# Bebra777228/PolGen-RVC

Hardware: AMD Instinct MI355X
Metric: real-time-factor (audio-sec/wall-sec) per GPU, 30s@16kHz RMVPE->48kHz (higher is better)
Workload: dtype f32 (conv products as 3 fp16 MFMAs of a hi/lo split, fp32 accumulate; fp32 elsewhere)

## Files before the change

### include/rvcx.h

```cpp
#ifndef RVCX_H
#define RVCX_H
#include <stdint.h>

#ifdef __cplusplus
extern "C" {
#endif

typedef struct rvcx_ctx rvcx_ctx;

typedef struct {
  const char* name;
  const void* data;
  int32_t dtype;
  int32_t ndim;
  int64_t shape[4];
} rvcx_tensor;

typedef struct {
  int32_t inter_channels, hidden_channels, filter_channels, n_heads, n_layers, kernel_size;
  int32_t n_resblocks;
  int32_t res_kernels[4];
  int32_t res_dilations[4][3];
  int32_t n_ups;
  int32_t up_rates[6], up_kernels[6];
// ... 242 lines not shown
int rvcx_index_features(rvcx_ctx*, int B, const float* wav_hd, int64_t n, int out_dim, float* feats_hd);
int64_t rvcx_kmeans_exhaustive(rvcx_ctx*);

int rvcx_debug_inject(rvcx_ctx*, int what);
double rvcx_flop_counter(rvcx_ctx*, int reset);
void* rvcx_stream(rvcx_ctx*);

int rvcx_op_fcpe_post(rvcx_ctx*, const float* raw_hd, int F_in, int p_len, double pitch, double f0_min, double f0_max,
                      int32_t* coarse, float* f0);
int rvcx_op_conv1d(rvcx_ctx*, const float* x, const float* w, const float* bias, const float* res,
                   float* y, int B, int Cin, int Tin, int Cout, int K, int stride, int dil,
                   int pad_left, int Tout, int groups, int pre_lrelu, float pre_slope, int act,
                   float act_slope, const int32_t* lens_in, const int32_t* lens_out);
int rvcx_op_resblock_pair(rvcx_ctx*, const float* x, const float* w1, const float* b1, const float* w2,
                          const float* b2, float* y, int B, int C, int T, int K, int dil, float slope, int fused,
                          const int32_t* lens);
int rvcx_op_resblock3(rvcx_ctx*, const float* x, const float* w1, const float* b1, const float* w2, const float* b2,
                      float* y, int B, int C, int T, const int32_t* dils, float slope, const int32_t* lens);
int rvcx_bench_resblock_pair(rvcx_ctx*, int B, int C, int T, int K, int dil, int fused, int iters,
                             float* ms_per_launch);
int rvcx_bench_conv1d(rvcx_ctx*, int B, int Cin, int Tin, int Cout, int K, int stride, int dil, int groups,
                      int iters, float* ms_per_launch);
int rvcx_conv_override(int tile, int variant, int splitk);
int rvcx_op_convtranspose1d(rvcx_ctx*, const float* x, const float* w, const float* bias, float* y,
                            int B, int Cin, int Tin, int Cout, int K, int stride, int pad,
                            int pre_lrelu, float pre_slope);
int rvcx_op_conv2d3x3(rvcx_ctx*, const float* x, const float* w, const float* bias, const float* res,
                      float* y, int B, int Cin, int H, int W, int Cout, int act);
int rvcx_op_convblock2d(rvcx_ctx*, const float* x, const float* w1, const float* b1, const float* w2, const float* b2,
                        const float* wsc, const float* bsc, float* y, int B, int Cin, int Cout, int H, int W,
                        const int32_t* rows);
int rvcx_op_convtranspose2d(rvcx_ctx*, const float* x, const float* w, const float* bias, float* y,
                            int B, int Cin, int H, int W, int Cout, int act);
int rvcx_op_attention(rvcx_ctx*, const float* q, const float* k, const float* v, float* out, int B,
                      int H, int D, int T, float scale, const float* emb_rel_k,
                      const float* emb_rel_v, int window, const int32_t* lens);
int rvcx_op_gemm_tm(rvcx_ctx*, const float* x_cf, const float* w, const float* bias, const float* res_tm, int B, int T,
                    int Cin, int Cout, int act, int exact_fp32, float* y_tm, float* y_cf, float* y_split);
int rvcx_bench_gemm(rvcx_ctx*, int64_t rows, int Cin, int Cout, int iters, float* ms_per_launch);
int rvcx_op_layernorm_tm(rvcx_ctx*, const float* x, const float* gamma, const float* beta, float* y, float* y_split,
                         int64_t rows, int C, float eps);
int rvcx_op_layernorm_c(rvcx_ctx*, const float* x, const float* gamma, const float* beta, float* y,
                        int B, int C, int T, float eps);
int rvcx_op_groupnorm_gelu(rvcx_ctx*, const float* x, const float* gamma, const float* beta, int B, int C, int T, float eps,
                           const int32_t* lens, float* y, float* stats, float* y_split);
int rvcx_op_hubert_conv0(rvcx_ctx*, const float* wav, const float* w, const float* gamma, const float* beta, int B, int C,
// ... 30 lines not shown
```

### polgen-rvc_amd/_lib.py

```python
from __future__ import annotations

import ctypes as C
import os
import threading
import types
from typing import Optional, Sequence

import numpy as np

_HERE = os.path.dirname(os.path.abspath(__file__))
LIB_PATH = os.environ.get("RVCX_LIBRARY") or os.path.join(_HERE, "librvcx.so")


class RvcxError(RuntimeError):
    pass


class Tensor(C.Structure):
    _fields_ = [("name", C.c_char_p), ("data", C.c_void_p), ("dtype", C.c_int32),
                ("ndim", C.c_int32), ("shape", C.c_int64 * 4)]


class SynthCfg(C.Structure):
    _fields_ = [("inter_channels", C.c_int32), ("hidden_channels", C.c_int32),
# ... 90 lines not shown
    Lb, Lx, Ls = int(Lb), int(Lx), int(Ls)
    assert y.shape == (Lb + Lx + Ls,) and b.shape == (Lx,)
    win = np.lib.stride_tricks.sliding_window_view(y[:Ls + Lx], Lx)
    den = np.sqrt((win * win).sum(1) + 1e-8)
    scores = (win @ b) / den
    mags = (np.abs(win) @ np.abs(b)) / den
    d = int(np.argmax(scores)) if offset is None else int(offset)
    out = y[d:d + Lb].copy()
    k = min(Lx, Lb)
    fin = np.sin(0.5 * np.pi * np.arange(Lx) / max(Lx - 1, 1)) ** 2
    out[:k] = y[d:d + k] * fin[:k] + b[:k] * (1.0 - fin[:k])
    return out, y[d + Lb:d + Lb + Lx].copy(), d, scores, mags


_lib = None

SYMBOLS = [
    "rvcx_create", "rvcx_destroy", "rvcx_last_error", "rvcx_version", "rvcx_load_hubert",
    "rvcx_load_rmvpe", "rvcx_index_exhaustive", "rvcx_load_crepe", "rvcx_crepe_frames", "rvcx_crepe_predict", "rvcx_op_crepe_decode", "rvcx_get_f0_crepe_x", "rvcx_load_fcpe", "rvcx_fcpe_f0", "rvcx_fcpe_frames", "rvcx_get_f0_fcpe_x", "rvcx_op_fcpe_post", "rvcx_load_synth", "rvcx_unload_synth", "rvcx_load_index", "rvcx_load_index_ivf",
    "rvcx_weights_regions", "rvcx_weights_adopt", "rvcx_weights_clone", "rvcx_rmvpe_f0", "rvcx_rmvpe_frames", "rvcx_rmvpe_mel", "rvcx_synth_infer_taps", "rvcx_hubert_features",
    "rvcx_hubert_frames", "rvcx_synth_infer", "rvcx_synth_infer_window", "rvcx_synth_dec_rf", "rvcx_synth_upp", "rvcx_index_blend",
    "rvcx_out_len", "rvcx_convert_batch", "rvcx_convert_batch_f64", "rvcx_micro_batch", "rvcx_bucket_length", "rvcx_last_micro_batches", "rvcx_last_cuts", "rvcx_noise_len",
    "rvcx_get_f0", "rvcx_get_f0_x", "rvcx_vc", "rvcx_vc_frames", "rvcx_last_timing",
    "rvcx_flop_counter", "rvcx_fp32_reruns", "rvcx_mem_info", "rvcx_conv_profile", "rvcx_conv_profile_csv", "rvcx_stream", "rvcx_op_conv1d", "rvcx_op_resblock_pair", "rvcx_bench_resblock_pair", "rvcx_bench_conv1d", "rvcx_conv_override", "rvcx_op_convtranspose1d",
    "rvcx_op_conv2d3x3", "rvcx_op_convblock2d", "rvcx_op_convtranspose2d", "rvcx_op_attention", "rvcx_op_layernorm_c",
    "rvcx_op_bigru", "rvcx_op_highpass", "rvcx_highpass_exact", "rvcx_convert_batch_ex", "rvcx_get_f0_x_ex", "rvcx_fp32_layers", "rvcx_fp32_pinned",
    "rvcx_gru_fallbacks", "rvcx_gru_publish_probe", "rvcx_debug_inject", "rvcx_f0_file_track", "rvcx_op_gemm_tm", "rvcx_op_layernorm_tm",
    "rvcx_resample_len", "rvcx_resample_f64", "rvcx_resample_f64_kind", "rvcx_bench_gemm", "rvcx_device_info",
    "rvcx_convert_submit", "rvcx_convert_wait", "rvcx_convert_poll", "rvcx_convert_inflight", "rvcx_ticket_lead_ms",
    "rvcx_synth_infer_head", "rvcx_op_sola", "rvcx_stream_open", "rvcx_stream_step", "rvcx_stream_reset", "rvcx_stream_close",
    "rvcx_stream_out_len", "rvcx_stream_noise_len", "rvcx_stream_frames",
    "rvcx_stream_open_io", "rvcx_stream_in_len", "rvcx_stream_delays", "rvcx_stream_resample_delay", "rvcx_stream_last_taps",
    "rvcx_stream_set", "rvcx_op_stream_resample",
    "rvcx_stream_open_fx", "rvcx_stream_out_channels", "rvcx_stream_set_fx", "rvcx_stream_last_fx_ms", "rvcx_op_stream_fx",
    "rvcx_fx_reverb_host",
    "rvcx_fx_chain", "rvcx_op_fx_highpass", "rvcx_op_fx_compressor", "rvcx_op_fx_gate", "rvcx_op_fx_reverb", "rvcx_op_fx_shelf",
    "rvcx_op_fx_chorus", "rvcx_op_fx_mix", "rvcx_fx_chunk", "rvcx_fx_last_passes", "rvcx_fx_cte", "rvcx_fx_delay",
    "rvcx_fx_coeffs", "rvcx_fx_highpass_host", "rvcx_fx_biquad_host", "rvcx_fx_follower_host", "rvcx_fx_compressor_host",
    "rvcx_fx_gate_host", "rvcx_fx_comb_host", "rvcx_fx_allpass_host", "rvcx_fx_chorus_host", "rvcx_fx_mix_host",
    "rvcx_op_groupnorm_gelu", "rvcx_op_hubert_conv0", "rvcx_op_sine_source", "rvcx_op_randn", "rvcx_op_reflect_pad",
    "rvcx_op_mel_post", "rvcx_op_decode_f0", "rvcx_op_avgpool2", "rvcx_op_gru_input", "rvcx_op_upsample_protect",
    "rvcx_kmeans", "rvcx_ivf_assign", "rvcx_kmeans_exhaustive", "rvcx_index_features",
    "rvcx_op_resblock3", "rvcx_flac_encode_bound", "rvcx_flac_encode_s16", "rvcx_flac_info", "rvcx_flac_decode_s32", "rvcx_flac_last_error",
]


def lib() -> C.CDLL:
# ... 530 lines not shown
    def resblock3(self, x, w1, b1, w2, b2, dils=(1, 3, 5), slope=0.1, lens=None):
        x, w1, w2 = f32(x), f32(w1), f32(w2)
        B, Cc, T = x.shape
        y = np.empty_like(x)
        b1 = None if b1 is None else f32(b1)
        b2 = None if b2 is None else f32(b2)
        d = i32(list(dils))
        li = i32(lens)
        self._ck(lib().rvcx_op_resblock3(self._h, _p(x), _p(w1), _p(b1), _p(w2), _p(b2), _p(y), B, Cc, T, _p(d, C.c_int32),
                                         C.c_float(slope), _p(li, C.c_int32)), "op_resblock3")
        return y

    def bench_resblock_pair(self, B, Cc, T, K, dil=1, fused=True, iters=10):
        ms = C.c_float(0)
        self._ck(lib().rvcx_bench_resblock_pair(self._h, B, Cc, T, K, dil, 1 if fused else 0, iters, C.byref(ms)),
                 "bench_resblock_pair")
        return ms.value, 4.0 * B * Cc * Cc * K * T / (ms.value * 1e-3) / 1e12

    @staticmethod
    def conv_override(tile=-1, variant=-1, splitk=-1):
        if lib().rvcx_conv_override(tile, variant, splitk) != 0:
            raise RvcxError("conv_override: " + (lib().rvcx_last_error(None) or b"").decode())

    def bench_conv1d(self, B, Cin, Tin, Cout, K, stride=1, dil=1, groups=1, iters=10):
        ms = C.c_float(0)
        self._ck(lib().rvcx_bench_conv1d(self._h, B, Cin, Tin, Cout, K, stride, dil, groups, iters, C.byref(ms)),
                 "bench_conv1d")
        pad = (K * dil - dil) // 2
        Tout = (Tin + 2 * pad - dil * (K - 1) - 1) // stride + 1
        flops = 2.0 * B * Cout * Tout * K * (Cin // groups)
        return ms.value, flops / (ms.value * 1e-3) / 1e12

    def convtranspose1d(self, x, w, bias=None, stride=1, pad=0, pre_lrelu=None):
        x, w = f32(x), f32(w)
        B, Cin, Tin = x.shape
        _, Cout, K = w.shape
        Tout = (Tin - 1) * stride - 2 * pad + K
        y = np.empty((B, Cout, Tout), np.float32)
        bias = None if bias is None else f32(bias)
        self._ck(lib().rvcx_op_convtranspose1d(self._h, _p(x), _p(w), _p(bias), _p(y), B, Cin, Tin, Cout, K,
                                               stride, pad, 0 if pre_lrelu is None else 1,
                                               C.c_float(0.0 if pre_lrelu is None else pre_lrelu)),
                 "op_convtranspose1d")
        return y

    def conv2d3x3(self, x, w, bias=None, res=None, act=0):
# ... 775 lines not shown

        def name(i):
            if kd[i] < 0:
                return f"conv_mfma_kernel<{bm[i]},{bn[i]}> (generic, strided/grouped)"
            if kd[i] == 600001:
                return "gemm_f32<64,64> (time-major Linear, exact fp32)"
            if kd[i] == 600002:
                return f"gemm_bd<{bm[i]},{bn[i]}> (time-major Linear, activations straight from global memory)"
            if kd[i] >= 600000:
                return f"gemm_h3<{bm[i]},{bn[i]}> (time-major Linear)"
            if kd[i] == 500003:
                return "resblock3 (whole k=3 ResBlock: three fused steps, persistent)"
            if kd[i] >= 500000:
                return f"resblock_pair<C={kd[i] - 500000},N1={bn[i]}> (c1 -> c2 -> +x fused)"
            if kd[i] >= 400000:
                c = kd[i] - 400000
                return f"conv_h3<{bm[i]},{bn[i]},{'linear' if c == 1 else 'stride2' if c == 2 else 'halo%d' % c}>"
            if kd[i] == 300001:
                return "conv_cout1 (vector FMA, Cout=1)"
            if kd[i] == 300003:
                return "conv_ws<64,320> (weight-stationary tile: a stage = one 16-channel chunk x all taps; K segments + finish)"
            if kd[i] == 300004:
                return "conv3_thin (3x3, C=16/32: streaming MFMA, B operand from global, DPP-shifted taps)"
            if kd[i] == 300002:
                return "convt_thin (ConvTranspose1d k4 s2, streaming MFMA + fused noise conv)"
            if kd[i] >= 300000:
                return "conv_cin1 (vector FMA, Cin=1)"
            if kd[i] >= 200000:
                return f"conv_fast_sb<{bm[i]},{bn[i]},stride2>"
            if kd[i] >= 100000:
                return f"conv_fast_sb<{bm[i]},{bn[i]},linear>"
            return f"conv_fast_sb<{bm[i]},{bn[i]},halo{kd[i] // 10}>"
        self._tile_names = [name(i) for i in range(N)]
        return [dict(tile=name(i), launches=int(la[i]), flops=float(fl[i]), ms=float(ms[i]))
                for i in range(N) if la[i] > 0]

    def conv_profile_csv(self) -> str:
        txt = (lib().rvcx_conv_profile_csv(self._h) or b"").decode()
        names = getattr(self, "_tile_names", None)
        if not names:
            return txt
        out = []
        for i, line in enumerate(txt.splitlines()):
            head, _, rest = line.partition(",")
            if i > 0 and head.isdigit() and int(head) < len(names):
                head = '"' + names[int(head)].split(" (")[0] + '"'
# ... 41 lines not shown
```

### polgen-rvc_amd/csrc/api_ops.hip

```cpp
#include "api_internal.h"
#include "h3_device.h"

using namespace rvcx;
using namespace rvcx::api;

static void to_host(Ctx& c, float* h, const float* d, size_t n) {
  RVCX_HIP(hipMemcpyAsync(h, d, n * sizeof(float), hipMemcpyDeviceToHost, c.stream));
  RVCX_HIP(hipStreamSynchronize(c.stream));
}
#define TEMP_REGION(C) WeightRegion tmp_region_; RegionScope tmp_scope_(*(C), tmp_region_)

extern "C" {

int rvcx_op_conv1d(rvcx_ctx* ctx, const float* x, const float* w, const float* bias, const float* res,
                   float* y, int B, int Cin, int Tin, int Cout, int K, int stride, int dil,
                   int pad_left, int Tout, int groups, int pre_lrelu, float pre_slope, int act,
                   float act_slope, const int32_t* lens_in, const int32_t* lens_out) {
  API_BEGIN(ctx)
  TEMP_REGION(C);
  size_t nx = (size_t)B * Cin * Tin, ny = (size_t)B * Cout * Tout;
  C->arena.reserve((nx + 2 * ny) * 4 + (64 << 20));
  C->arena.reset();
  ConvW L = make_conv(*C, w, bias, Cout, Cin / groups, K, groups, true);
  float* dx = to_dev(*C, x, nx);
// ... 211 lines not shown
  RVCX_HIP(hipEventCreate(&e0));
  RVCX_HIP(hipEventCreate(&e1));
  RVCX_HIP(hipEventRecord(e0, C->stream));
  for (int i = 0; i < iters; ++i) once();
  RVCX_HIP(hipEventRecord(e1, C->stream));
  RVCX_HIP(hipEventSynchronize(e1));
  float ms = 0.f;
  RVCX_HIP(hipEventElapsedTime(&ms, e0, e1));
  *ms_per_launch = ms / iters;
  (void)hipEventDestroy(e0);
  (void)hipEventDestroy(e1);
  C->arena.reset();
  API_END
}

int rvcx_conv_override(int tile, int variant, int splitk) {
  REQUIRE_DEBUG(nullptr, "rvcx_conv_override")
  rvcx::g_conv_override.tile = tile;
  rvcx::g_conv_override.variant = variant;
  rvcx::g_conv_override.splitk = splitk;
  return 0;
}

int rvcx_bench_conv1d(rvcx_ctx* ctx, int B, int Cin, int Tin, int Cout, int K, int stride, int dil, int groups,
                      int iters, float* ms_per_launch) {
  REQUIRE_DEBUG(ctx, "rvcx_bench_conv1d")
  API_BEGIN(ctx)
  TEMP_REGION(C);
  const int pad = (K * dil - dil) / 2;
  const int Tout = (Tin + 2 * pad - dil * (K - 1) - 1) / stride + 1;
  size_t nx = (size_t)B * Cin * Tin, ny = (size_t)B * Cout * Tout;
  C->arena.reserve((nx + 2 * ny) * 4 + (64 << 20));
  C->arena.reset();
  std::vector<float> w((size_t)Cout * (Cin / groups) * K), bias((size_t)Cout, 0.1f);
  for (size_t i = 0; i < w.size(); ++i) w[i] = (float)((i * 2654435761u) % 2001) / 1000.f - 1.f;
  ConvW L = make_conv(*C, w.data(), bias.data(), Cout, Cin / groups, K, groups, true);
  float* dx = C->arena.alloc<float>(nx);
  float* dy = C->arena.alloc<float>(ny);
  float* dr = C->arena.alloc<float>(ny);
  launch_randn(dx, nx, 1, 0, C->stream);
  launch_randn(dr, ny, 2, 0, C->stream);
  ConvArgs a = conv1d_args(L, dx, dy, B, Tin, Tout, stride, dil, pad);
  conv_set_res(a, dr, Cout, Tout);
  a.pre_act = ACT_LRELU;
  a.pre_slope = 0.1f;
  C->conv(a);
// ... 644 lines not shown
```

### polgen-rvc_amd/csrc/conv.h

```cpp
#pragma once
#include "common.h"

namespace rvcx {

enum Act { ACT_NONE = 0, ACT_LRELU = 1, ACT_RELU = 2, ACT_GELU = 3, ACT_TANH = 4, ACT_SIGMOID = 5 };
enum OutMode { OUT_NORMAL = 0, OUT_SHUF1D = 1, OUT_SHUF2D = 2, OUT_TRANSPOSED = 3 };
enum Acc2 { ACC2_NONE = 0, ACC2_SET = 1, ACC2_ADD = 2, ACC2_ADD_DIV = 3 };

struct ConvArgs {
  const float* x = nullptr;
  const float* w = nullptr;
  const void* w_h3 = nullptr;
  const void* x_split = nullptr;
  void* y_split = nullptr;
  const float* bias = nullptr;
  const float* res = nullptr;
  float* y = nullptr;
  float* y2 = nullptr;
  const int* lens_in = nullptr;
  const int* lens_out = nullptr;
  int B = 1;
  int Cin_g = 0, Cin_gp = 0, Cout_g = 0, Cout_gp = 0, groups = 1;
  int Tin = 0;
  int Nout = 0;
// ... 101 lines not shown

struct ConvProfile {
  static constexpr int kMaxTiles = 72;
  long launches[kMaxTiles] = {0};
  double flops[kMaxTiles] = {0};
  double ms[kMaxTiles] = {0};
  int bm[kMaxTiles] = {0}, bn[kMaxTiles] = {0}, halo[kMaxTiles] = {0};
};
void conv_profile_begin();
void conv_profile_end(ConvProfile* out);
const char* conv_profile_csv();
void conv_init();
void launch_conv(ConvArgs a, hipStream_t stream);
int launch_conv_fast(ConvArgs& a, hipStream_t stream);
void conv_fast_describe(ConvProfile* p);
int launch_conv_h3(ConvArgs& a, int halo, int off_min, hipStream_t stream);
bool convt_thin_ok(const ConvArgs& a);
void launch_convt_thin(const ConvArgs& a, hipStream_t stream);
void convt_thin_init();
constexpr int kConvtThinSlot = 61;
bool conv3_thin_ok(const ConvArgs& a);
void launch_conv3_thin(const ConvArgs& a, hipStream_t stream);
constexpr int kConv3ThinSlot = 59;
bool conv_deep_ok(const ConvArgs& a);
void launch_conv_deep(const ConvArgs& a, hipStream_t stream);
constexpr int kConvDeepSlot = 63;
bool conv_h3_enabled();
bool conv_h3_configured();
bool conv_h3_split_ok(const ConvArgs& a);
void launch_splitk_finish(const ConvArgs& a, hipStream_t stream);
void conv_h3_describe(ConvProfile* p);
struct ConvOverride { int tile = -1, variant = -1, splitk = -1; };
extern ConvOverride g_conv_override;
void conv_fast_init();
double conv_flops(const ConvArgs& a);

int conv_cin_pad(int cin_g);
int conv_cout_pad(int cout_g);
std::vector<float> pack_conv_weight(const float* w, int cout, int cin_g, int k, int groups);
struct PolyPhase1d {
  std::vector<float> w;
  std::vector<float> bias;
  int taps = 0;
  int pad = 0;
  int cout_total = 0;
};
// ... 5 lines not shown
```

### polgen-rvc_amd/csrc/conv.hip

```cpp
#include "conv.h"
#include "conv_device.h"
#include "gemm.h"

#include <algorithm>
#include <cmath>

namespace rvcx {

template <int BM, int BN, int WR, int WC>
__global__ __launch_bounds__(256) void conv_mfma_kernel(const ConvArgs a) {
  constexpr int WM = BM / (32 * WR), WN = BN / (32 * WC);
  static_assert(WR * WC == 4 && WM >= 1 && WN >= 1, "bad tile");
  extern __shared__ float smem[];
  float* As = smem;
  float* Bs = smem + a.kk_chunk * a.ci_chunk * BM;

  const int tid = threadIdx.x, lane = tid & 63, wave = tid >> 6;
  const int wr = wave / WC, wc = wave % WC;
  const int i = lane & 31, h = lane >> 5;
  const int b = blockIdx.z;
  const int mt_per_g = (a.Cout_gp + BM - 1) / BM;
  const int g = blockIdx.y / mt_per_g, mt = blockIdx.y % mt_per_g;
  const int co0 = mt * BM;
  const int n0 = blockIdx.x * BN;
// ... 146 lines not shown

void conv_profile_begin() {
  g_prof.clear();
  g_prof_on = true;
}

static std::string g_prof_csv;
const char* conv_profile_csv() { return g_prof_csv.c_str(); }

void conv_profile_end(ConvProfile* out) {
  g_prof_on = false;
  g_prof_csv = "tile,B,cin,cout,k,stride,nout,gflop,ms,tflops\n";
  for (int t = 0; t < kNumTiles; ++t) {
    out->bm[t] = kTiles[t].bm;
    out->bn[t] = kTiles[t].bn;
    out->halo[t] = -1;
  }
  conv_fast_describe(out);
  conv_h3_describe(out);
  resblock_pair_describe(out);
  out->bm[kBlock3Slot] = 64;
  out->bn[kBlock3Slot] = resblock3_n1(64);
  out->halo[kBlock3Slot] = 500003;
  gemm_describe(out);
  for (auto& r : g_prof) {
    RVCX_HIP(hipEventSynchronize(r.b));
    float ms = 0.f;
    RVCX_HIP(hipEventElapsedTime(&ms, r.a, r.b));
    out->launches[r.tile] += 1;
    out->flops[r.tile] += r.flops;
    out->ms[r.tile] += ms;
    char line[256];
    snprintf(line, sizeof line, "%d,%d,%d,%d,%d,%d,%d,%.3f,%.4f,%.1f\n", r.tile, r.B, r.cin, r.cout, r.k, r.stride,
             r.nout, r.flops / 1e9, ms, r.flops / (ms * 1e-3) / 1e12);
    g_prof_csv += line;
    (void)hipEventDestroy(r.a);
    (void)hipEventDestroy(r.b);
  }
  g_prof.clear();
}

void conv_launch_pair(const PairArgs& a, double flops, hipStream_t stream) {
  if (!g_prof_on) {
    launch_resblock_pair(a, stream);
    return;
  }
// ... 2 lines not shown
  RVCX_HIP(hipEventCreate(&rec.b));
  rec.tile = resblock_pair_slot(a.C);
  rec.flops = flops;
  rec.cin = a.C; rec.cout = a.C; rec.k = a.k; rec.nout = a.T; rec.stride = a.dil; rec.B = a.B;
  RVCX_HIP(hipEventRecord(rec.a, stream));
  launch_resblock_pair(a, stream);
  RVCX_HIP(hipEventRecord(rec.b, stream));
  g_prof.push_back(rec);
}

void conv_launch_block3(const Block3Args& a, double flops, hipStream_t stream) {
  if (!g_prof_on) {
    launch_resblock3(a, stream);
    return;
  }
  ProfRec rec;
  RVCX_HIP(hipEventCreate(&rec.a));
  RVCX_HIP(hipEventCreate(&rec.b));
  rec.tile = kBlock3Slot;
  rec.flops = flops;
  rec.cin = a.C; rec.cout = a.C; rec.k = 3; rec.nout = a.T; rec.stride = 135; rec.B = a.B;
  RVCX_HIP(hipEventRecord(rec.a, stream));
  launch_resblock3(a, stream);
  RVCX_HIP(hipEventRecord(rec.b, stream));
  g_prof.push_back(rec);
}

void conv_launch_gemm(const GemmArgs& a, double flops, hipStream_t stream) {
  if (!g_prof_on) {
    launch_gemm(a, stream);
    return;
  }
  ProfRec rec;
  RVCX_HIP(hipEventCreate(&rec.a));
  RVCX_HIP(hipEventCreate(&rec.b));
  rec.flops = flops;
  rec.cin = a.cin; rec.cout = a.cout; rec.k = 1; rec.nout = (int)a.rows; rec.stride = 1; rec.B = (int)(a.rows / a.T);
  RVCX_HIP(hipEventRecord(rec.a, stream));
  rec.tile = launch_gemm(a, stream);
  RVCX_HIP(hipEventRecord(rec.b, stream));
  g_prof.push_back(rec);
}

void launch_conv(ConvArgs a, hipStream_t stream) {
  RVCX_CHECK(a.Cin_gp % 2 == 0 && a.Cout_gp % 32 == 0, "conv: unpadded weights");
  RVCX_CHECK(a.Nout > 0 && a.B > 0, "conv: empty problem");
// ... 101 lines not shown
```

### polgen-rvc_amd/csrc/ctx.h

```cpp
#pragma once
#include <memory>

#include "common.h"
#include "conv.h"
#include "gemm.h"

namespace rvcx {

struct SynthModel;
struct RmvpeModel;
struct FcpeModel;
struct CrepeModel;
struct HubertModel;
struct IndexData;

class WeightRegion {
 public:
  static constexpr size_t kChunkBytes = (size_t)32 << 20;
  static constexpr int kMaxFlags = 4096;
  static constexpr size_t kHeaderBytes = kMaxFlags;
  WeightRegion() {
    flags_.reset(new uint8_t[kMaxFlags]);
    std::memset(flags_.get(), 0, kMaxFlags);
  }
// ... 202 lines not shown
    for (auto& p : splitk_buf)
      if (p) {
        (void)hipFree(p);
        p = nullptr;
      }
    splitk_items = items;
  }
  void pair_on(const PairArgs& a, hipStream_t s) {
    const double f = 2.0 * 2.0 * a.B * (double)a.C * a.C * a.k * a.T;
    flops += f;
    PairArgs b = a;
    b.ovf = dev_err;
    b.seq = ++launch_seq;
    conv_launch_pair(b, f, s);
  }
  void block3_on(const Block3Args& a, hipStream_t s) {
    const double f = 3.0 * 2.0 * 2.0 * a.B * (double)a.C * a.C * 3 * a.T;
    flops += f;
    Block3Args b = a;
    b.ovf = dev_err;
    b.seq = ++launch_seq;
    conv_launch_block3(b, f, s);
  }
  void gemm_on(GemmArgs a, hipStream_t s) {
    const double f = 2.0 * (double)a.rows * a.cout * a.cin;
    flops += f;
    a.ovf = dev_err;
    a.seq = ++launch_seq;
    {
      const int si = (s == stream2) ? 1 : (s == aux[0] ? 2 : (s == aux[1] ? 3 : 0));
      if (!splitk_buf[si]) RVCX_HIP(hipMalloc(&splitk_buf[si], kSplitKFloats * splitk_items * sizeof(float)));
      a.part = splitk_buf[si];
      a.part_cap = kSplitKFloats * splitk_items;
    }
    conv_launch_gemm(a, f, s);
  }
  void conv(const ConvArgs& a) { conv_on(a, stream); }
  void conv_on(ConvArgs a, hipStream_t s) {
    flops += conv_flops(a);
    const int si = (s == stream2) ? 1 : (s == aux[0] ? 2 : (s == aux[1] ? 3 : 0));
    if (!splitk_buf[si]) RVCX_HIP(hipMalloc(&splitk_buf[si], kSplitKFloats * splitk_items * sizeof(float)));
    a.part = splitk_buf[si];
    a.part_cap = kSplitKFloats * splitk_items;
    a.part_cap_item = kSplitKFloats;
    a.ovf = dev_err;
    a.seq = ++launch_seq;
// ... 69 lines not shown
```

### polgen-rvc_amd/csrc/rmvpe.hip

```cpp
#include <cmath>

#include "models.h"
#include "ops.h"

namespace rvcx {

namespace {

constexpr int N_FFT = 1024, HOP = 160, N_MELS = 128;
constexpr double SR = 16000.0, FMIN = 30.0, FMAX = 8000.0;

std::vector<float> stft_basis() {
  const int nb = N_FFT / 2 + 1;
  std::vector<float> w((size_t)2 * nb * N_FFT);
  for (int k = 0; k < nb; ++k)
    for (int n = 0; n < N_FFT; ++n) {
      const double ang = 2.0 * M_PI * (double)(k * n) / (double)N_FFT;
      const float win = (float)(0.5 - 0.5 * std::cos(2.0 * M_PI * (double)n / (double)N_FFT));
      w[(size_t)k * N_FFT + n] = (float)std::cos(ang) * win;
      w[(size_t)(nb + k) * N_FFT + n] = (float)(-std::sin(ang)) * win;
    }
  return w;
}

// ... 166 lines not shown

namespace {
struct Map2 {
  float* p = nullptr;
  long bs = 0;
  int C = 0, H = 0, Wp = 0;
};

void run_block(Ctx& c, const RmvpeModel::Block& b, const Map2& x, const Map2& y, float* tmp1, float* tmp2, int B,
               hipStream_t s, const int* lens) {
  const int H = x.H, Wp = x.Wp;
  ConvArgs a = conv2d_args(b.c1, x.p, tmp1, B, H, Wp);
  a.x_bs = x.bs;
  a.act = ACT_RELU;
  a.lens_in = a.lens_out = lens;
  ConvArgs a2 = conv2d_args(b.c2, tmp1, y.p, B, H, Wp);
  a2.lens_in = a2.lens_out = lens;
  const bool ws = conv_deep_ok(a) && conv_deep_ok(a2);
  const bool split = !ws && (long)H * Wp >= 20000 && conv_h3_split_ok(a) && conv_h3_split_ok(a2) && !getenv("RVCX_NO_SPLIT");
  if (split) {
    a.y_split = tmp1;
    a.y = nullptr;
  }
  c.conv_on(a, s);
  const float* res = x.p;
  long res_bs = x.bs;
  if (b.has_sc) {
    a = conv2d_args(b.sc, x.p, tmp2, B, H, Wp);
    a.x_bs = x.bs;
    a.lens_in = a.lens_out = lens;
    c.conv_on(a, s);
    res = tmp2;
    res_bs = (long)b.cout * H * Wp;
  }
  a = a2;
  if (split) a.x_split = tmp1;
  a.act = ACT_RELU;
  a.res = res;
  a.res_bs = res_bs;
  a.res_cs = H * Wp;
  a.y_bs = y.bs;
  c.conv_on(a, s);
}
}

void rmvpe_block_op(Ctx& c, const ConvW& c1, const ConvW& c2, const ConvW* sc, const float* x, float* y, float* tmp1,
                    float* tmp2, int B, int H, int Wp, const int* rows, hipStream_t s) {
  RmvpeModel::Block blk;
  blk.c1 = c1;
  blk.c2 = c2;
  blk.cin = c1.cin;
  blk.cout = c1.cout;
  if (sc) {
    blk.sc = *sc;
    blk.has_sc = true;
  }
  const int* d_len = nullptr;
  if (rows) {
    std::vector<int> v(B);
    for (int b = 0; b < B; ++b) v[b] = rows[b] * Wp;
    d_len = dev_ints_many(c.arena, {v}, s)[0];
  }
  Map2 xm{const_cast<float*>(x), (long)blk.cin * H * Wp, blk.cin, H, Wp};
  Map2 ym{y, (long)blk.cout * H * Wp, blk.cout, H, Wp};
  run_block(c, blk, xm, ym, tmp1, tmp2, B, s, d_len);
// ... 176 lines not shown
```

Baseline: 1228.

## Fuse thin RMVPE ConvBlockRes into one kernel with LDS-resident intermediate

Adds a fused kernel for RMVPE residual conv blocks with 16/32 channels. It runs conv1 into an LDS band (with halo rows), then conv2 plus the 1x1 shortcut or identity residual, all in one launch. This removes the intermediate split-tensor round trip through global memory and two or three kernel launches per block. In exchange it recomputes halo rows per band, and band height is picked by a heuristic bounded by available LDS. It is enabled by default and can be turned off with an env switch.

New measurement: 1240, median of 6. Within noise of the previous version (+1.0%).

```diff
diff --git a/include/rvcx.h b/include/rvcx.h
--- a/include/rvcx.h
+++ b/include/rvcx.h
@@ -288,6 +288,7 @@
 int rvcx_bench_conv1d(rvcx_ctx*, int B, int Cin, int Tin, int Cout, int K, int stride, int dil, int groups,
                       int iters, float* ms_per_launch);
 int rvcx_conv_override(int tile, int variant, int splitk);
+int rvcx_convblock_fused(int on);
 int rvcx_op_convtranspose1d(rvcx_ctx*, const float* x, const float* w, const float* bias, float* y,
                             int B, int Cin, int Tin, int Cout, int K, int stride, int pad,
                             int pre_lrelu, float pre_slope);
diff --git a/polgen-rvc_amd/_lib.py b/polgen-rvc_amd/_lib.py
--- a/polgen-rvc_amd/_lib.py
+++ b/polgen-rvc_amd/_lib.py
@@ -136,7 +136,7 @@
     "rvcx_hubert_frames", "rvcx_synth_infer", "rvcx_synth_infer_window", "rvcx_synth_dec_rf", "rvcx_synth_upp", "rvcx_index_blend",
     "rvcx_out_len", "rvcx_convert_batch", "rvcx_convert_batch_f64", "rvcx_micro_batch", "rvcx_bucket_length", "rvcx_last_micro_batches", "rvcx_last_cuts", "rvcx_noise_len",
     "rvcx_get_f0", "rvcx_get_f0_x", "rvcx_vc", "rvcx_vc_frames", "rvcx_last_timing",
-    "rvcx_flop_counter", "rvcx_fp32_reruns", "rvcx_mem_info", "rvcx_conv_profile", "rvcx_conv_profile_csv", "rvcx_stream", "rvcx_op_conv1d", "rvcx_op_resblock_pair", "rvcx_bench_resblock_pair", "rvcx_bench_conv1d", "rvcx_conv_override", "rvcx_op_convtranspose1d",
+    "rvcx_flop_counter", "rvcx_fp32_reruns", "rvcx_mem_info", "rvcx_conv_profile", "rvcx_conv_profile_csv", "rvcx_stream", "rvcx_op_conv1d", "rvcx_op_resblock_pair", "rvcx_bench_resblock_pair", "rvcx_bench_conv1d", "rvcx_conv_override", "rvcx_convblock_fused", "rvcx_op_convtranspose1d",
     "rvcx_op_conv2d3x3", "rvcx_op_convblock2d", "rvcx_op_convtranspose2d", "rvcx_op_attention", "rvcx_op_layernorm_c",
     "rvcx_op_bigru", "rvcx_op_highpass", "rvcx_highpass_exact", "rvcx_convert_batch_ex", "rvcx_get_f0_x_ex", "rvcx_fp32_layers", "rvcx_fp32_pinned",
     "rvcx_gru_fallbacks", "rvcx_gru_publish_probe", "rvcx_debug_inject", "rvcx_f0_file_track", "rvcx_op_gemm_tm", "rvcx_op_layernorm_tm",
@@ -713,6 +713,13 @@
         if lib().rvcx_conv_override(tile, variant, splitk) != 0:
             raise RvcxError("conv_override: " + (lib().rvcx_last_error(None) or b"").decode())
 
+    @staticmethod
+    def convblock_fused(on=-1) -> int:
+        r = lib().rvcx_convblock_fused(int(on))
+        if r < 0:
+            raise RvcxError("convblock_fused: " + (lib().rvcx_last_error(None) or b"").decode())
+        return int(r)
+
     def bench_conv1d(self, B, Cin, Tin, Cout, K, stride=1, dil=1, groups=1, iters=10):
         ms = C.c_float(0)
         self._ck(lib().rvcx_bench_conv1d(self._h, B, Cin, Tin, Cout, K, stride, dil, groups, iters, C.byref(ms)),
@@ -1534,6 +1541,8 @@
                 return "conv_ws<64,320> (weight-stationary tile: a stage = one 16-channel chunk x all taps; K segments + finish)"
             if kd[i] == 300004:
                 return "conv3_thin (3x3, C=16/32: streaming MFMA, B operand from global, DPP-shifted taps)"
+            if kd[i] == 300005:
+                return "conv3_thin_block (fused ConvBlockRes, C=16/32: conv1 -> LDS -> conv2 + shortcut / residual, one launch)"
             if kd[i] == 300002:
                 return "convt_thin (ConvTranspose1d k4 s2, streaming MFMA + fused noise conv)"
             if kd[i] >= 300000:
diff --git a/polgen-rvc_amd/csrc/api_ops.hip b/polgen-rvc_amd/csrc/api_ops.hip
--- a/polgen-rvc_amd/csrc/api_ops.hip
+++ b/polgen-rvc_amd/csrc/api_ops.hip
@@ -257,6 +257,11 @@
   return 0;
 }
 
+int rvcx_convblock_fused(int on) {
+  if (on == 0 || on == 1 || on >= 100) REQUIRE_DEBUG(nullptr, "rvcx_convblock_fused")
+  return rvcx::convblock_fused_switch(on);
+}
+
 int rvcx_bench_conv1d(rvcx_ctx* ctx, int B, int Cin, int Tin, int Cout, int K, int stride, int dil, int groups,
                       int iters, float* ms_per_launch) {
   REQUIRE_DEBUG(ctx, "rvcx_bench_conv1d")
diff --git a/polgen-rvc_amd/csrc/conv.h b/polgen-rvc_amd/csrc/conv.h
--- a/polgen-rvc_amd/csrc/conv.h
+++ b/polgen-rvc_amd/csrc/conv.h
@@ -147,6 +147,28 @@
 bool conv3_thin_ok(const ConvArgs& a);
 void launch_conv3_thin(const ConvArgs& a, hipStream_t stream);
 constexpr int kConv3ThinSlot = 59;
+struct BlockThinArgs {
+  const float* x = nullptr;
+  float* y = nullptr;
+  const void* w1 = nullptr;
+  const void* w2 = nullptr;
+  const void* wsc = nullptr;
+  const float* b1 = nullptr;
+  const float* b2 = nullptr;
+  const float* bsc = nullptr;
+  const int* lens = nullptr;
+  int B = 1, Cin = 0, Cout = 0, H = 0, Wp = 0;
+  long x_bs = 0, y_bs = 0;
+  int* ovf = nullptr;
+  int* ovf_layer = nullptr;
+  int seq = 0;
+  int R = 0, nbands = 0;
+};
+int convblock_fused_switch(int on);
+bool convblock_thin_ok(const ConvArgs& c1, const ConvArgs& c2, const ConvArgs* sc);
+void launch_convblock_thin(BlockThinArgs a, hipStream_t stream);
+void conv_launch_block_thin(const BlockThinArgs& a, double flops, hipStream_t stream);
+constexpr int kConvBlockThinSlot = 65;
 bool conv_deep_ok(const ConvArgs& a);
 void launch_conv_deep(const ConvArgs& a, hipStream_t stream);
 constexpr int kConvDeepSlot = 63;
diff --git a/polgen-rvc_amd/csrc/conv.hip b/polgen-rvc_amd/csrc/conv.hip
--- a/polgen-rvc_amd/csrc/conv.hip
+++ b/polgen-rvc_amd/csrc/conv.hip
@@ -192,6 +192,9 @@
   out->bm[kBlock3Slot] = 64;
   out->bn[kBlock3Slot] = resblock3_n1(64);
   out->halo[kBlock3Slot] = 500003;
+  out->bm[kConvBlockThinSlot] = 32;
+  out->bn[kConvBlockThinSlot] = 30;
+  out->halo[kConvBlockThinSlot] = 300005;
   gemm_describe(out);
   for (auto& r : g_prof) {
     RVCX_HIP(hipEventSynchronize(r.b));
@@ -240,6 +243,23 @@
   rec.cin = a.C; rec.cout = a.C; rec.k = 3; rec.nout = a.T; rec.stride = 135; rec.B = a.B;
   RVCX_HIP(hipEventRecord(rec.a, stream));
   launch_resblock3(a, stream);
+  RVCX_HIP(hipEventRecord(rec.b, stream));
+  g_prof.push_back(rec);
+}
+
+void conv_launch_block_thin(const BlockThinArgs& a, double flops, hipStream_t stream) {
+  if (!g_prof_on) {
+    launch_convblock_thin(a, stream);
+    return;
+  }
+  ProfRec rec;
+  RVCX_HIP(hipEventCreate(&rec.a));
+  RVCX_HIP(hipEventCreate(&rec.b));
+  rec.tile = kConvBlockThinSlot;
+  rec.flops = flops;
+  rec.cin = a.Cin; rec.cout = a.Cout; rec.k = 9; rec.nout = a.H * a.Wp; rec.stride = 1; rec.B = a.B;
+  RVCX_HIP(hipEventRecord(rec.a, stream));
+  launch_convblock_thin(a, stream);
   RVCX_HIP(hipEventRecord(rec.b, stream));
   g_prof.push_back(rec);
 }
diff --git a/polgen-rvc_amd/csrc/convblock_thin.hip b/polgen-rvc_amd/csrc/convblock_thin.hip
--- /dev/null
+++ b/polgen-rvc_amd/csrc/convblock_thin.hip
@@ -0,0 +1,393 @@
+#include <algorithm>
+#include <cstdlib>
+#include <mutex>
+#include <utility>
+
+#include "conv.h"
+#include "conv_device.h"
+#include "h3_device.h"
+
+namespace rvcx {
+
+namespace {
+
+constexpr int kTileN = 30;
+constexpr int kWaves = 16;
+constexpr int kThreads = 64 * kWaves;
+constexpr int kSlab = 4 * 32 * 16;
+
+template <class F, int... I>
+__device__ __forceinline__ void static_for_impl(F&& f, std::integer_sequence<int, I...>) {
+  (f(std::integral_constant<int, I>{}), ...);
+}
+template <int N, class F>
+__device__ __forceinline__ void static_for(F&& f) {
+  static_for_impl(f, std::make_integer_sequence<int, N>{});
+}
+
+__device__ __forceinline__ half8 shl1(half8 v) {
+  uint4 u = __builtin_bit_cast(uint4, v);
+#if defined(__HIP_DEVICE_COMPILE__)
+  u.x = (unsigned)__builtin_amdgcn_update_dpp(0, (int)u.x, 0x130, 0xf, 0xf, false);
+  u.y = (unsigned)__builtin_amdgcn_update_dpp(0, (int)u.y, 0x130, 0xf, 0xf, false);
+  u.z = (unsigned)__builtin_amdgcn_update_dpp(0, (int)u.z, 0x130, 0xf, 0xf, false);
+  u.w = (unsigned)__builtin_amdgcn_update_dpp(0, (int)u.w, 0x130, 0xf, 0xf, false);
+#endif
+  return __builtin_bit_cast(half8, u);
+}
+
+template <int NCH, int KS>
+__device__ __forceinline__ void load_weights(uint4* dst, const void* img, int tid) {
+  const H3Rsrc wres = h3_rsrc(img, KS * NCH * kSlab);
+  for (int e = tid; e < NCH * KS * 2 * 64; e += kThreads) {
+    const int l = e & 63, f = e >> 6;
+    const int op = f & 1, ck = f >> 1, chunk = ck / KS, kk = ck - chunk * KS;
+    const int ii = l & 31, hh = l >> 5;
+    dst[e] = h3_load4(wres, (kk * NCH + chunk) * kSlab + ((op * 2 + hh) * 32 + ii) * 16);
+  }
+}
+
+__device__ __forceinline__ void split8(const float (&v)[8], half8& hi, half8& lo, bool& ovf) {
+  static_for<8>([&](auto k_) {
+    constexpr int k = k_;
+    ovf |= !(fabsf(v[k]) < kH3ActLimit);
+    const _Float16 vh = (_Float16)v[k];
+    hi[k] = vh;
+    lo[k] = (_Float16)((v[k] - (float)vh) * kH3Scale);
+  });
+}
+
+template <int NCH>
+__device__ __forceinline__ f32x16 taps3x3(const uint4* W, int lz, const half8 (&bq)[3][NCH][2]) {
+  f32x16 acc;
+  static_for<16>([&](auto r_) { acc[(int)r_] = 0.f; });
+  half8 swh = __builtin_bit_cast(half8, W[0 * 64 + lz]), swl = __builtin_bit_cast(half8, W[1 * 64 + lz]);
+  static_for<NCH>([&](auto c_) {
+    static_for<3>([&](auto dy_) {
+      constexpr int c = c_, dy = dy_;
+      half8 xh = bq[dy][c][0], xl = bq[dy][c][1];
+      static_for<3>([&](auto dx_) {
+        constexpr int dx = dx_, f = c * 9 + dy * 3 + dx;
+        half8 nwh = swh, nwl = swl;
+        if constexpr (f + 1 < NCH * 9) {
+          nwh = __builtin_bit_cast(half8, W[((f + 1) * 2 + 0) * 64 + lz]);
+          nwl = __builtin_bit_cast(half8, W[((f + 1) * 2 + 1) * 64 + lz]);
+        }
+        const half8 wh = swh * (_Float16)(1.f / kH3Scale);
+        acc = h3_mfma(swh, xh, acc);
+        acc = h3_mfma(wh, xl, acc);
+        acc = h3_mfma(swl, xh, acc);
+        if constexpr (dx < 2) {
+          xh = shl1(xh);
+          xl = shl1(xl);
+        }
+#if defined(__HIP_DEVICE_COMPILE__)
+        __builtin_amdgcn_sched_barrier(0);
+#endif
+        swh = nwh;
+        swl = nwl;
+      });
+    });
+  });
+  return acc;
+}
+
+template <int CIN, int CMID, bool SC>
+__global__ __launch_bounds__(kThreads) void convblock_thin_kernel(const BlockThinArgs a) {
+  constexpr int NC1 = CIN / 16, NC2 = CMID / 16;
+  extern __shared__ uint4 lds[];
+  uint4* const W1 = lds;
+  uint4* const W2 = W1 + NC1 * 9 * 2 * 64;
+  uint4* const WS = W2 + NC2 * 9 * 2 * 64;
+  uint4* const Mid = WS + (SC ? NC1 * 2 * 64 : 0);
+  const int tid = threadIdx.x, lane = tid & 63, wave = tid >> 6;
+  load_weights<NC1, 9>(W1, a.w1, tid);
+  load_weights<NC2, 9>(W2, a.w2, tid);
+  if constexpr (SC) load_weights<NC1, 1>(WS, a.wsc, tid);
+
+  const int Wp = a.Wp, HW = a.H * Wp;
+  const int NP = (a.R + 2) * Wp + 2;
+  const int total = a.nbands * a.B;
+  const int G = gridDim.x;
+  const int wg = (G & 7) == 0 ? (int)(blockIdx.x & 7) * (G >> 3) + (int)(blockIdx.x >> 3) : (int)blockIdx.x;
+  constexpr float inv = 1.f / kH3Scale;
+  bool ovf = false;
+
+  for (int t = wg; t < total; t += G) {
+    const int b = t / a.nbands, band = t - b * a.nbands;
+    const int r0 = band * a.R, r1 = min(a.H, r0 + a.R);
+    const int o0 = r0 * Wp, o1 = r1 * Wp;
+    const int m0 = o0 - Wp - 1, m1 = o1 + Wp + 1;
+    const int len = a.lens ? a.lens[b] : 0x7fffffff;
+    const int lim = min(len, HW);
+    const H3Rsrc xr = h3_rsrc(a.x + (long)b * a.x_bs, CIN * HW * 4);
+    __syncthreads();
+
+    const int nt1 = (m1 - m0 + kTileN - 1) / kTileN;
+    for (int tl = wave; tl < nt1; tl += kWaves) {
+      const int pm = m0 + tl * kTileN;
+      int lz = lane;
+      asm volatile("" : "+v"(lz));
+      const int i = lz & 31, h = lz >> 5;
+      f32x16 acc;
+      static_for<16>([&](auto r_) { acc[(int)r_] = 0.f; });
+      if (pm < lim && pm + 32 > 0) {
+        half8 bq[3][NC1][2];
+        static_for<3>([&](auto dy_) {
+          constexpr int dy = dy_;
+          const int q = pm - 1 + i + (dy - 1) * Wp;
+          const bool ok = q >= 0 && q < lim;
+          static_for<NC1>([&](auto c_) {
+            constexpr int c = c_;
+            float v[8];
+            static_for<8>([&](auto k_) {
+              constexpr int k = k_;
+              v[k] = h3_load1(xr, ok ? ((c * 16 + 8 * h + k) * HW + q) * 4 : kH3Oob);
+            });
+            split8(v, bq[dy][c][0], bq[dy][c][1], ovf);
+          });
+        });
+        acc = taps3x3<NC1>(W1, lz, bq);
+        static_for<16>([&](auto r_) { acc[(int)r_] *= inv; });
+      }
+      const int nn = pm + i;
+      if (i < kTileN && nn < m1) {
+        bool live = nn >= 0 && nn < lim;
+        if (live) {
+          const int col = nn % Wp;
+          live = col != 0 && col != Wp - 1;
+        }
+        char* base = reinterpret_cast<char*>(Mid) + (long)(nn - m0) * 16 + 8 * h;
+        static_for<CMID / 8>([&](auto g_) {
+          constexpr int g = g_, cg = 8 * g;
+          typedef _Float16 half4 __attribute__((ext_vector_type(4)));
+          half4 hi, lo;
+          static_for<4>([&](auto q_) {
+            constexpr int q = q_;
+            float v = acc[4 * g + q] + (a.b1 ? a.b1[cg + 4 * h + q] : 0.f);
+            v = v > 0.f ? v : 0.f;
+            v = live ? v : 0.f;
+            ovf |= !(fabsf(v) < kH3ActLimit);
+            const _Float16 vh = (_Float16)v;
+            hi[q] = vh;
+            lo[q] = (_Float16)((v - (float)vh) * kH3Scale);
+          });
+          constexpr int e_hi = ((cg >> 4) * 2 + 0) * 2 + (g & 1), e_lo = ((cg >> 4) * 2 + 1) * 2 + (g & 1);
+          *reinterpret_cast<half4*>(base + (long)e_hi * NP * 16) = hi;
+          *reinterpret_cast<half4*>(base + (long)e_lo * NP * 16) = lo;
+        });
+      }
+    }
+    __syncthreads();
+
+    const int nt2 = (o1 - o0 + kTileN - 1) / kTileN;
+    for (int tl = wave; tl < nt2; tl += kWaves) {
+      const int p0 = o0 + tl * kTileN;
+      int lz = lane;
+      asm volatile("" : "+v"(lz));
+      const int i = lz & 31, h = lz >> 5;
+      const int nn = p0 + i;
+      f32x16 acc, accs;
+      static_for<16>([&](auto r_) {
+        acc[(int)r_] = 0.f;
+        accs[(int)r_] = 0.f;
+      });
+      if (p0 < len) {
+        {
+          half8 bq[3][NC2][2];
+          static_for<3>([&](auto dy_) {
+            constexpr int dy = dy_;
+            const int idx = min(nn - 1 + (dy - 1) * Wp - m0, m1 - m0 - 1);
+            static_for<NC2>([&](auto c_) {
+              constexpr int c = c_;
+              bq[dy][c][0] = __builtin_bit_cast(half8, Mid[((c * 2 + 0) * 2 + h) * NP + idx]);
+              bq[dy][c][1] = __builtin_bit_cast(half8, Mid[((c * 2 + 1) * 2 + h) * NP + idx]);
+            });
+          });
+          acc = taps3x3<NC2>(W2, lz, bq);
+          static_for<16>([&](auto r_) { acc[(int)r_] *= inv; });
+        }
+        if constexpr (SC) {
+          const bool ok = nn < lim;
+          static_for<NC1>([&](auto c_) {
+            constexpr int c = c_;
+            float v[8];
+            static_for<8>([&](auto k_) {
+              constexpr int k = k_;
+              v[k] = h3_load1(xr, ok ? ((c * 16 + 8 * h + k) * HW + nn) * 4 : kH3Oob);
+            });
+            half8 xh, xl;
+            split8(v, xh, xl, ovf);
+            const half8 swh = __builtin_bit_cast(half8, WS[(c * 2 + 0) * 64 + lz]);
+            const half8 swl = __builtin_bit_cast(half8, WS[(c * 2 + 1) * 64 + lz]);
+            const half8 wh = swh * (_Float16)(1.f / kH3Scale);
+            accs = h3_mfma(swh, xh, accs);
+            accs = h3_mfma(wh, xl, accs);
+            accs = h3_mfma(swl, xh, accs);
+          });
+          static_for<16>([&](auto r_) { accs[(int)r_] *= inv; });
+        }
+      }
+      if (i < kTileN && nn < o1) {
+        bool live = nn < len;
+        {
+          const int col = nn % Wp;
+          live = live && col != 0 && col != Wp - 1;
+        }
+        float* yb = a.y + (long)b * a.y_bs + nn;
+        const float* rb = a.x + (long)b * a.x_bs + nn;
+        static_for<2>([&](auto half_) {
+          constexpr int rbase = 8 * half_;
+          float bv[8], rv[8];
+          static_for<8>([&](auto q_) {
+            constexpr int q = q_, r = rbase + q;
+            const int co = 4 * h + (r & 3) + 8 * (r >> 2);
+            const int cc = co < CMID ? co : 0;
+            bv[q] = a.b2 ? a.b2[cc] : 0.f;
+            if constexpr (SC) {
+              const float vs = accs[r] + (a.bsc ? a.bsc[cc] : 0.f);
+              rv[q] = fmaxf(vs, vs * 1.f) + 0.f;
+            } else {
+              rv[q] = rb[(long)cc * HW];
+            }
+          });
+          static_for<8>([&](auto q_) {
+            constexpr int q = q_, r = rbase + q;
+            const int co = 4 * h + (r & 3) + 8 * (r >> 2);
+            if (co < CMID) {
+              float v = acc[r] + bv[q];
+              v = fmaxf(v, v * 0.f) + rv[q];
+              yb[(long)co * HW] = live ? v : 0.f;
+            }
+          });
+        });
+      }
+    }
+  }
+  if (ovf) report_h3_overflow(a.ovf, a.ovf_layer, a.seq);
+}
+
+size_t weight_bytes(int cin, int cmid, bool sc) {
+  return (size_t)((cin / 16) * 9 * 2 * 64 + (cmid / 16) * 9 * 2 * 64 + (sc ? (cin / 16) * 2 * 64 : 0)) * 16;
+}
+size_t lds_bytes(int cin, int cmid, bool sc, int R, int Wp) {
+  return weight_bytes(cin, cmid, sc) + (size_t)((R + 2) * Wp + 2) * cmid * 4;
+}
+
+struct Dev {
+  int ncu = 256, lds = 64 << 10;
+};
+const Dev& dev_info() {
+  static const Dev d = [] {
+    Dev v;
+    int dev = 0, n = 0;
+    if (hipGetDevice(&dev) == hipSuccess) {
+      if (hipDeviceGetAttribute(&n, hipDeviceAttributeMultiprocessorCount, dev) == hipSuccess && n > 0) v.ncu = n;
+      if (hipDeviceGetAttribute(&n, hipDeviceAttributeMaxSharedMemoryPerBlock, dev) == hipSuccess && n > 0) v.lds = n;
+    }
+    v.lds = std::min(v.lds, 160 << 10);
+    return v;
+  }();
+  return d;
+}
+
+int max_band_rows(int cin, int cmid, bool sc, int Wp) {
+  const long room = (long)dev_info().lds - (long)weight_bytes(cin, cmid, sc);
+  if (room <= 0) return 0;
+  const long np = room / (cmid * 4);
+  return (int)std::max(0L, (np - 2) / Wp - 2);
+}
+
+template <int CIN, int CMID, bool SC>
+void launch(const BlockThinArgs& a, int grid, size_t lds, hipStream_t stream) {
+  static std::mutex mu;
+  static uint64_t done = 0;
+  int dev = 0;
+  RVCX_HIP(hipGetDevice(&dev));
+  {
+    std::lock_guard<std::mutex> g(mu);
+    if (!((done >> (dev & 63)) & 1)) {
+      RVCX_HIP(hipFuncSetAttribute(reinterpret_cast<const void*>(convblock_thin_kernel<CIN, CMID, SC>),
+                                   hipFuncAttributeMaxDynamicSharedMemorySize, dev_info().lds));
+      done |= 1ull << (dev & 63);
+    }
+  }
+  hipLaunchKernelGGL((convblock_thin_kernel<CIN, CMID, SC>), dim3(grid), dim3(kThreads), lds, stream, a);
+}
+
+int g_fused = -1;
+int g_rows = 0;
+
+}
+
+int convblock_fused_switch(int on) {
+  static std::mutex mu;
+  std::lock_guard<std::mutex> g(mu);
+  if (g_fused < 0) g_fused = (!getenv("RVCX_CONVBLOCK_FUSED") || atoi(getenv("RVCX_CONVBLOCK_FUSED")) != 0) ? 1 : 0;
+  if (on == 0 || on == 1) {
+    g_fused = on;
+    g_rows = 0;
+  } else if (on >= 100) {
+    g_fused = 1;
+    g_rows = on - 100;
+  }
+  return g_fused;
+}
+
+bool convblock_thin_ok(const ConvArgs& c1, const ConvArgs& c2, const ConvArgs* sc) {
+  if (convblock_fused_switch(-1) == 0) return false;
+  if (!conv3_thin_ok(c1) || !conv3_thin_ok(c2)) return false;
+  if (!c1.y_split || !c2.x_split || c1.x_split || c2.y_split || !c2.y || !c2.res) return false;
+  if (c1.act != ACT_RELU || c2.act != ACT_RELU || c1.acc2_mode != ACC2_NONE || c2.acc2_mode != ACC2_NONE) return false;
+  const int cin = c1.Cin_g, cm = c1.Cout_g, Wp = c1.rowpitch, HW = c1.Nout;
+  if (c2.Cin_g != cm || c2.Cout_g != cm || !(cm == 16 || cm == 32) || c1.Cout_gp != 32 || c2.Cout_gp != 32) return false;
+  if (c2.rowpitch != Wp || c2.Nout != HW || HW % Wp != 0 || c1.Tin != HW || c2.Tin != HW) return false;
+  if (c1.zero_wp != Wp || c2.zero_wp != Wp || c1.x_cs != HW || c2.y_cs != HW || c2.res_cs != HW) return false;
+  if (c1.lens_in != c1.lens_out || c2.lens_in != c1.lens_in || c2.lens_out != c1.lens_in || c1.B != c2.B) return false;
+  if (sc) {
+    if (cin == cm || !sc->w_h3 || !conv_h3_enabled() || sc->ksize != 1 || sc->groups != 1 || sc->stride != 1) return false;
+    if (sc->Cin_g != cin || sc->Cin_gp != cin || sc->Cout_g != cm || sc->Cout_gp != 32 || sc->x != c1.x || sc->x_bs != c1.x_bs) return false;
+    if (sc->act != ACT_NONE || sc->pre_act != ACT_NONE || sc->res || sc->out_mode != OUT_NORMAL || sc->acc2_mode != ACC2_NONE) return false;
+    if (sc->lens_in != c1.lens_in || sc->lens_out != c1.lens_in || sc->zero_wp != Wp || sc->Nout != HW || sc->x_cs != HW) return false;
+    if (c2.res != sc->y) return false;
+  } else {
+    if (cin != cm || c2.res != c1.x || c2.res_bs != c1.x_bs) return false;
+  }
+  return max_band_rows(cin, cm, sc != nullptr, Wp) >= 2;
+}
+
+void launch_convblock_thin(BlockThinArgs a, hipStream_t stream) {
+  const bool sc = a.wsc != nullptr;
+  const int rmax = max_band_rows(a.Cin, a.Cout, sc, a.Wp);
+  RVCX_CHECK(rmax >= 1, "convblock_thin: no band fits LDS");
+  const int ncu = dev_info().ncu;
+  int best_r = 1, best_rounds = 1;
+  long best_cost = -1;
+  for (int r = 1; r <= std::min(rmax, a.H); ++r) {
+    const long bands = (long)cdiv(a.H, r) * a.B;
+    const int rounds = (int)((bands + ncu - 1) / ncu);
+    const long cost = (long)rounds * (2 * r + 3);
+    if (best_cost < 0 || cost <= best_cost) {
+      best_cost = cost;
+      best_r = r;
+      best_rounds = rounds;
+    }
+  }
+  if (g_rows > 0) {
+    best_r = std::min({g_rows, rmax, a.H});
+    best_rounds = (int)(((long)cdiv(a.H, best_r) * a.B + ncu - 1) / ncu);
+  }
+  a.R = best_r;
+  a.nbands = cdiv(a.H, best_r);
+  const long bands = (long)a.nbands * a.B;
+  const int grid = (int)((bands + best_rounds - 1) / best_rounds);
+  const size_t lds = lds_bytes(a.Cin, a.Cout, sc, a.R, a.Wp);
+  if (a.Cin == 16 && a.Cout == 16 && !sc) launch<16, 16, false>(a, grid, lds, stream);
+  else if (a.Cin == 32 && a.Cout == 32 && !sc) launch<32, 32, false>(a, grid, lds, stream);
+  else if (a.Cin == 32 && a.Cout == 16 && sc) launch<32, 16, true>(a, grid, lds, stream);
+  else if (a.Cin == 16 && a.Cout == 32 && sc) launch<16, 32, true>(a, grid, lds, stream);
+  else fail("convblock_thin: unsupported channel counts");
+  RVCX_HIP(hipGetLastError());
+}
+
+}
diff --git a/polgen-rvc_amd/csrc/ctx.h b/polgen-rvc_amd/csrc/ctx.h
--- a/polgen-rvc_amd/csrc/ctx.h
+++ b/polgen-rvc_amd/csrc/ctx.h
@@ -248,6 +248,13 @@
     b.seq = ++launch_seq;
     conv_launch_block3(b, f, s);
   }
+  void block_thin_on(BlockThinArgs a, double f, int nlaunch, hipStream_t s) {
+    flops += f;
+    a.ovf = dev_err;
+    a.seq = launch_seq + 1;
+    launch_seq += nlaunch;
+    conv_launch_block_thin(a, f, s);
+  }
   void gemm_on(GemmArgs a, hipStream_t s) {
     const double f = 2.0 * (double)a.rows * a.cout * a.cin;
     flops += f;
diff --git a/polgen-rvc_amd/csrc/rmvpe.hip b/polgen-rvc_amd/csrc/rmvpe.hip
--- a/polgen-rvc_amd/csrc/rmvpe.hip
+++ b/polgen-rvc_amd/csrc/rmvpe.hip
@@ -212,25 +212,50 @@
     a.y_split = tmp1;
     a.y = nullptr;
   }
-  c.conv_on(a, s);
   const float* res = x.p;
   long res_bs = x.bs;
+  ConvArgs asc;
   if (b.has_sc) {
-    a = conv2d_args(b.sc, x.p, tmp2, B, H, Wp);
-    a.x_bs = x.bs;
-    a.lens_in = a.lens_out = lens;
-    c.conv_on(a, s);
+    asc = conv2d_args(b.sc, x.p, tmp2, B, H, Wp);
+    asc.x_bs = x.bs;
+    asc.lens_in = asc.lens_out = lens;
     res = tmp2;
     res_bs = (long)b.cout * H * Wp;
   }
-  a = a2;
-  if (split) a.x_split = tmp1;
-  a.act = ACT_RELU;
-  a.res = res;
-  a.res_bs = res_bs;
-  a.res_cs = H * Wp;
-  a.y_bs = y.bs;
+  if (split) a2.x_split = tmp1;
+  a2.act = ACT_RELU;
+  a2.res = res;
+  a2.res_bs = res_bs;
+  a2.res_cs = H * Wp;
+  a2.y_bs = y.bs;
+  if (split && convblock_thin_ok(a, a2, b.has_sc ? &asc : nullptr)) {
+    BlockThinArgs f;
+    f.x = x.p;
+    f.y = y.p;
+    f.w1 = a.w_h3;
+    f.w2 = a2.w_h3;
+    f.b1 = a.bias;
+    f.b2 = a2.bias;
+    if (b.has_sc) {
+      f.wsc = asc.w_h3;
+      f.bsc = asc.bias;
+    }
+    f.lens = lens;
+    f.B = B;
+    f.Cin = b.c1.cin;
+    f.Cout = b.c1.cout;
+    f.H = H;
+    f.Wp = Wp;
+    f.x_bs = x.bs;
+    f.y_bs = y.bs;
+    f.ovf_layer = a.ovf_layer;
+    const double fl = conv_flops(a) + (b.has_sc ? conv_flops(asc) : 0.0) + conv_flops(a2);
+    c.block_thin_on(f, fl, b.has_sc ? 3 : 2, s);
+    return;
+  }
   c.conv_on(a, s);
+  if (b.has_sc) c.conv_on(asc, s);
+  c.conv_on(a2, s);
 }
 }
 
```
